# lrm2017/Fastest_Image_Pattern_Matching

Measured on AMD Instinct MI355X. Metric: template matches/sec + ms/search, 4024×3036 src ±180°; HBM GB/s vs roofline, higher is better.
Workload: dtype u8

## Files before the change

fastest_image_pattern_matching_amd/csrc/fpm_kernels.hip:

```cpp
#include <float.h>
#include <stdio.h>
#include <stdlib.h>
#include <limits.h>

#include <map>
#include <mutex>
#include <type_traits>
#include <utility>

#include "../../include/fpm.h"
#include "fpm_kernels.h"
#include "fpm_model.h"
#include "fpm_rrect.h"

static void ensure_lds_attr(const void* fn, size_t bytes) {
    if (bytes <= 65536) return;
    int dev = 0;
    (void)hipGetDevice(&dev);
    static std::mutex mu;
    static std::map<std::pair<int, const void*>, size_t> done;
    std::lock_guard<std::mutex> lock(mu);
    size_t& cur = done[std::make_pair(dev, fn)];
    if (bytes <= cur) return;
    (void)hipFuncSetAttribute(fn, hipFuncAttributeMaxDynamicSharedMemorySize, (int)bytes);
// ... 3549 lines not shown
        else { slot = item / nband; band = item - slot * nband; }
        const int T0 = band * kBandRows, rb = min(kBandRows, th - T0), nsrc = rb + 6;
        __syncthreads();
        if (NK > 0) {
            const bool in_roi = lane < 2 * txn;
            if (DMA) {
                dma_rows(item, SB);
                flush();
                asm volatile("s_waitcnt vmcnt(0)" ::: "memory");
            } else {
            if (!PFR) load_rows(item);
            flush();
#pragma unroll
            for (int i = 0; i < kStageRows; ++i) {
                const int r = wv + 4 * i;
                if (r < nsrc && lane < q4)
                    *(uint4*)(SB + (size_t)r * SBp + 16 * lane) = in_roi ? pv[i] : make_uint4(kRoiFlip, kRoiFlip, kRoiFlip, kRoiFlip);
            }
            }
            if (band != a_band) {
                a_band = band;
                if (tid < kBandRows) lts[tid] = tid < rb ? (uint32_t)a.tsum[T0 + tid] : 0u;
                if (kMmaRows * mt < rb) {
                    const int8_t* ap = a.tmpl8 + (size_t)(T0 + kMmaRows * mt + n) * a.tp8 + 16 * g;
#pragma unroll
                    for (int k = 0; k < NA; ++k)
                        if (k < a.nk) Areg[k] = *(const fpm_v4i*)(ap + 64 * k);
                }
            }
            if (PFR && item + 1 < it_hi) load_rows(item + 1);
        } else if (MODE != 3) {
            if (tid < kBandRows) lts[tid] = tid < rb ? (uint32_t)a.tsum[T0 + tid] : 0u;
            const uint8_t* rsrc = a.roi + (size_t)slot * a.roi_stride;
            for (int c0 = 0; c0 < q4; c0 += 64) {
                const int c = c0 + lane;
                for (int i0 = 0; i0 < kStageRows; i0 += kStageBatch) {
                    uint4 v[kStageBatch];
#pragma unroll
                    for (int i = 0; i < kStageBatch; ++i) {
                        const int r = wv + 4 * (i0 + i);
                        const int R = T0 + r;
                        v[i] = (r < nsrc && c < 2 * txn)
                                   ? *(const uint4*)(rsrc + ((size_t)((R >> 5) * txn + (c >> 1)) << 10) + (R & 31) * ROI_T + 16 * (c & 1))
                                   : make_uint4(kRoiFlip, kRoiFlip, kRoiFlip, kRoiFlip);
                    }
#pragma unroll
                    for (int i = 0; i < kStageBatch; ++i) {
                        const int r = wv + 4 * (i0 + i);
                        if (r < nsrc && c < q4) *(uint4*)(SB + (size_t)r * SBp + 16 * c) = v[i];
                    }
                }
            }
        }
        __syncthreads();
        if (RS >= 3 && MODE != 7 && wv != 2 && kMmaRows * nt < nsrc) {
            int ln = lane;
            asm volatile("" : "+v"(ln));
            const int g3 = ln >> 4, n3 = ln & 15, row = kMmaRows * nt + n3;
            const int sr = row < nsrc ? row : 0;
            uint32_t* rw = (uint32_t*)(SB + (size_t)sr * SBp);
            if (npad > 0) {
                if (g3 < npad) rw[nwr + g3] = kRoiFlip;
                if (g3 + 4 < npad) rw[nwr + g3 + 4] = kRoiFlip;
            }
            const int wr = tw >> 2;
            const uint32_t l0 = rw[0], l1 = rw[1], x0 = rw[wr], x1 = rw[wr + 1], x2 = rw[wr + 2];
            uint32_t s1, s2;
            tile_row_sums<RS == 4>((const uint8_t*)rw + 16 * g3, a.nk, n3, s1, s2);
            s2 = (uint32_t)__shfl((int)s2, n3 + 16 * (n3 >> 2), 64);
            const uint32_t e0 = __builtin_amdgcn_alignbyte(x1, x0, (uint32_t)tw) ^ 0x80808080u;
            const uint32_t e1 = __builtin_amdgcn_alignbyte(x2, x1, (uint32_t)tw) ^ 0x80808080u;
            const uint64_t lo = (uint64_t)(l0 ^ 0x80808080u) | ((uint64_t)(l1 ^ 0x80808080u) << 32);
            const uint64_t hi = (uint64_t)e0 | ((uint64_t)e1 << 32);
            const int nf = min(6, 64 * a.nk - tw);
#pragma unroll
            for (int h = 0; h < 2; ++h) {
                const int dx = g3 + 4 * h;
                if (dx < 7 && row < nsrc) {
                    uint32_t q1, q2;
                    window_edges(lo, hi, dx, nf, q1, q2);
                    wi[row * 7 + dx] = s1 - q1;
                    wq[row * 7 + dx] = s2 - q2;
                }
            }
        }
        if (RS == 1 && MODE != 7 && tid < 4 * nsrc) {
            const int r = tid >> 2, qq = tid & 3;
            const int per = (nwr + 3) >> 2, k0 = qq * per, k1 = min(nwr, k0 + per);
            const uint32_t* row = (const uint32_t*)(SB + (size_t)r * SBp);
            uint32_t s1 = 0, s2 = 0;
            int k = k0;
            for (; k + 8 <= k1; k += 8) {
                uint32_t x[8];
#pragma unroll
                for (int u = 0; u < 8; ++u) x[u] = row[k + u] ^ 0x80808080u;
#pragma unroll
                for (int u = 0; u < 8; ++u) {
                    s1 = __builtin_amdgcn_udot4(x[u], 0x01010101u, s1, false);
                    s2 = __builtin_amdgcn_udot4(x[u], x[u], s2, false);
                }
            }
            for (; k < k1; ++k) {
                const uint32_t x = row[k] ^ 0x80808080u;
                s1 = __builtin_amdgcn_udot4(x, 0x01010101u, s1, false);
                s2 = __builtin_amdgcn_udot4(x, x, s2, false);
            }
            const uint32_t l0 = row[0] ^ 0x80808080u, l1 = row[1] ^ 0x80808080u;
            const int wr = tw >> 2;
            const uint32_t x0 = row[wr], x1 = row[wr + 1], x2 = row[wr + 2];
            const uint32_t e0 = __builtin_amdgcn_alignbyte(x1, x0, (uint32_t)tw) ^ 0x80808080u;
            const uint32_t e1 = __builtin_amdgcn_alignbyte(x2, x1, (uint32_t)tw) ^ 0x80808080u;
            s1 += (uint32_t)__builtin_amdgcn_mov_dpp((int)s1, 0xB1, 0xF, 0xF, false);
            s2 += (uint32_t)__builtin_amdgcn_mov_dpp((int)s2, 0xB1, 0xF, 0xF, false);
            s1 += (uint32_t)__builtin_amdgcn_mov_dpp((int)s1, 0x4E, 0xF, 0xF, false);
            s2 += (uint32_t)__builtin_amdgcn_mov_dpp((int)s2, 0x4E, 0xF, 0xF, false);
#pragma unroll
            for (int h = 0; h < 2; ++h) {
                const int dx = qq + 4 * h;
                if (dx < 7) {
                    const uint32_t ml0 = dx >= 4 ? 0xffffffffu : (1u << (8 * dx)) - 1u;
                    const uint32_t ml1 = dx <= 4 ? 0u : (1u << (8 * (dx - 4))) - 1u;
                    const uint32_t mr0 = dx >= 4 ? 0u : ~((1u << (8 * dx)) - 1u);
                    const uint32_t mr1 = dx <= 4 ? 0xffffu : dx == 5 ? 0xff00u : 0u;
                    const uint32_t a0 = l0 & ml0, a1 = l1 & ml1, b0 = e0 & mr0, b1 = e1 & mr1;
                    uint32_t q1 = __builtin_amdgcn_udot4(a0, 0x01010101u, 0u, false);
                    q1 = __builtin_amdgcn_udot4(a1, 0x01010101u, q1, false);
                    q1 = __builtin_amdgcn_udot4(b0, 0x01010101u, q1, false);
                    q1 = __builtin_amdgcn_udot4(b1, 0x01010101u, q1, false);
                    uint32_t q2 = __builtin_amdgcn_udot4(a0, a0, 0u, false);
                    q2 = __builtin_amdgcn_udot4(a1, a1, q2, false);
                    q2 = __builtin_amdgcn_udot4(b0, b0, q2, false);
                    q2 = __builtin_amdgcn_udot4(b1, b1, q2, false);
                    wi[r * 7 + dx] = s1 - q1;
                    wq[r * 7 + dx] = s2 - q2;
                }
            }
        }
        __syncthreads();
        auto partials = [&]() {
            if (MODE == 6 || tid >= 4 * 49) return;
            const int pr = tid >> 1, half = tid & 1;
            const int h = pr / 49, k = pr - h * 49;
            const int chunk = (T0 >> 4) + h;
            const int tlo = kMmaRows * h, thi = min(tlo + kMmaRows, rb);
            const bool ok = chunk < a.nchunk && tlo < thi;
            const int pdy = k / 7, ddx = k - pdy * 7;
            const int t0 = tlo + 8 * half, n8 = ok ? min(8, thi - t0) : 0;
            uint32_t s1 = 0, x[8], y[8];
#pragma unroll
            for (int u = 0; u < 8; ++u) {
                const int i = (t0 + u + pdy) * 7 + ddx;
                x[u] = u < n8 ? wi[i] : 0u;
                y[u] = u < n8 ? wq[i] : 0u;
            }
            uint64_t s2 = 0;
#pragma unroll
            for (int u = 0; u < 8; ++u) { s1 += x[u]; s2 += y[u]; }
            s1 += (uint32_t)__builtin_amdgcn_mov_dpp((int)s1, 0xB1, 0xF, 0xF, false);
            const uint32_t lo = (uint32_t)s2, hi = (uint32_t)(s2 >> 32);
            s2 += (uint64_t)(uint32_t)__builtin_amdgcn_mov_dpp((int)lo, 0xB1, 0xF, 0xF, false) |
                  ((uint64_t)(uint32_t)__builtin_amdgcn_mov_dpp((int)hi, 0xB1, 0xF, 0xF, false) << 32);
            if (ok && half == 0) {
                uint32_t kk = (uint32_t)k;
                asm volatile("" : "+v"(kk));
                const uint32_t wo = ((uint32_t)slot * (uint32_t)a.nchunk + (uint32_t)chunk) * 49u + kk;
                a.wsum[wo] = s1;
                a.wsq[wo] = s2;
            }
        };
        const bool active = kMmaRows * mt < rb && kMmaRows * nt < nsrc;
        if (FPM_CORR_PRIO == 1) __builtin_amdgcn_s_setprio(1);
        if (MODE != 2 && active) {
            int sr = kMmaRows * nt + n;
            if (sr >= nsrc) sr = 0;
            const uint8_t* bp = SB + (size_t)sr * SBp + 16 * g;
            fpm_v4i acc[7];
            if (FPM_CORR_PRIO == 2) __builtin_amdgcn_s_setprio(1);
            if (NK > 0)
                band_mfma_regs<NA>(Areg, bp, a.nk, acc);
            else
                band_mfma_ga(a.tmpl8 + (size_t)(T0 + kMmaRows * mt + n) * a.tp8 + 16 * g, bp, a.nk, acc);
            if (FPM_CORR_PRIO == 2) __builtin_amdgcn_s_setprio(0);
            uint32_t* rs_out = a.rowsum + (((size_t)th * 49 + 3) & ~(size_t)3) * slot + (size_t)T0 * 49;
            const uint32_t kFix = 16384u * (uint32_t)tw;
            int t0 = kMmaRows * mt + 4 * g;
            asm volatile("" : "+v"(t0));
            const int s_ = kMmaRows * nt + n;
            const uint4 ts4 = *(const uint4*)(lts + t0);
#pragma unroll
            for (int r = 0; r < 4; ++r) {
                const int t = t0 + r, dy = s_ - t;
                if (t < rb && s_ < nsrc && dy >= 0 && dy < 7) {
                    const uint32_t ts = r == 0 ? ts4.x : r == 1 ? ts4.y : r == 2 ? ts4.z : ts4.w;
                    if (MODE == 5) {
                        uint32_t x = ts;
#pragma unroll
                        for (int d = 0; d < 7; ++d) x += (uint32_t)acc[d][r];
                        if (x == 0x9e3779b9u && a.W < 0) rs_out[t] = x;
                        continue;
                    }
                    const uint32_t o = (uint32_t)(t * 49 + dy * 7);
                    if (SE) {
#pragma unroll
                        for (int d = 0; d < 7; ++d) rsb[o + d] = (uint32_t)acc[d][r] + 128u * (wi[s_ * 7 + d] + ts) - kFix;
                        continue;
                    }
#pragma unroll
                    for (int d = 0; d < 7; ++d) rs_out[o + d] = (uint32_t)acc[d][r] + 128u * (wi[s_ * 7 + d] + ts) - kFix;
                }
            }
        }
        if (FPM_CORR_PRIO == 1) __builtin_amdgcn_s_setprio(0);
        partials();
        if (SE) { pv_slot = slot; pv_T0 = T0; pv_rb = rb; }
    }
    if (SE && pv_slot >= 0) {
        __syncthreads();
        flush();
    }
}

__device__ __forceinline__ CandState cand_step_state(CandState s, int n3, const AngleNode* nodes, double thr, int W,
                                                     int H, int mark_reached0, const float* score, const int* mx,
                                                     const int* my, const AngleNode* next_nodes = nullptr,
                                                     int jj = 0, AngleNode* next_nd = nullptr, int nnext = 1) {
    int imax = 0;
    double big = -1;
    for (int k = 0; k < n3; ++k)
        if ((double)score[k] > big) { imax = k; big = score[k]; }
    if ((double)score[imax] < thr) {
        s.alive = 0;
        return s;
    }
    const int child = s.node * n3 + imax;
    const AngleNode nd = nodes[child];
    if (next_nodes)
        for (int k = 0; k < nnext; ++k) next_nd[k] = next_nodes[child * n3 + jj + k];
    const F2 sc = f2((W - 1) / 2.0f, (H - 1) / 2.0f);
    const F2 r0 = rotate_pt(f2(s.lt.x * 2, s.lt.y * 2), sc, nd.c, nd.s);
    const F2 pad = f2(r0.x - 3, r0.y - 3);
    F2 p = f2((float)((double)mx[imax] + pad.x), (float)((double)my[imax] + pad.y));
    p = rotate_pt(p, sc, nd.cn, nd.sn);
    s.lt = p;
    s.node = child;
    s.reached0 = mark_reached0;
    return s;
}

struct SmallLayout {
    int sbp, tbp, rh, u, tab, sum, rs, sc, ts, total;
};
__host__ __device__ inline int isqrt_ceil(int n) {
    int d = 0;
    while ((d + 1) * (d + 1) <= n) ++d;
    return d * d == n ? d : d + 1;
}
__host__ __device__ inline int small_footprint_bound(int rw, int rh) {
    const int d = isqrt_ceil((rw - 1) * (rw - 1) + (rh - 1) * (rh - 1)) + 2;
    return ((d + 16) * (d + 6) + 15) & ~15;
}
__host__ __device__ inline SmallLayout small_layout(int tw, int th, int nw = 4) {
    SmallLayout L;
    L.sbp = roi_pitch_calc(tw);
    L.tbp = tmpl_lds_pitch(64 * ((tw + 63) / 64));
    L.rh = th + 6;
    const int th16 = (th + kMmaRows - 1) / kMmaRows * kMmaRows;
    L.u = ((L.rh + 16) * L.sbp + 15) & ~15;
    const int fb = small_footprint_bound(tw + 6, th + 6);
    const int fp = fb < nw * ROI_FT ? fb : nw * ROI_FT;
    const int ub = th16 * L.tbp > fp ? th16 * L.tbp : fp;
    L.tab = L.u + ub;
    L.sum = L.tab + 4 * (2 * L.sbp + 2 * ((L.rh + 3) & ~3));
    const int rs_size = 4 * kBandRows * 49;
    const int after_sums = L.sum + 4 * (2 * L.rh + 2 * 7 * L.rh) + 8 * 49 * 2;
    if (th16 * L.tbp + rs_size <= L.sum - L.u) {
        L.rs = L.u + th16 * L.tbp;
        L.sc = after_sums;
    } else {
        L.rs = after_sums;
        L.sc = L.rs + rs_size;
    }
    L.ts = L.sc + 4 * 64;
    L.total = L.ts + 4 * th16;
    return L;
}
constexpr int kSmallLdsMax = 72 * 1024;
bool roi_small_fits(int tw, int th) { return th <= 256 && small_layout(tw, th).total <= kSmallLdsMax; }
size_t roi_small_lds(int tw, int th) { return (size_t)small_layout(tw, th).total; }

template <int MODE, int WPE = 3, bool PROL = false, int NT = 256>
__global__ __launch_bounds__(NT) __attribute__((amdgpu_waves_per_eu(WPE))) void k_roi_small(RoiArgs a) {
    constexpr int NW = NT / 64;
    extern __shared__ __attribute__((aligned(16))) uint8_t smem[];
    const int tw = a.tw, th = a.th, RW = tw + 6, RH = th + 6, W = a.W, H = a.H;
    const SmallLayout LY = small_layout(tw, th, NW);
    const int SBp = LY.sbp, TBp = LY.tbp;
    uint8_t* SB = smem;
    uint8_t* TB = smem + LY.u;
    uint8_t* FTall = smem + LY.u;
    int32_t* lad = (int32_t*)(smem + LY.tab);
    int32_t* lbd = lad + SBp;
    int32_t* lx0 = lbd + SBp;
    int32_t* ly0 = lx0 + ((RH + 3) & ~3);
    uint32_t* rall = (uint32_t*)(smem + LY.sum);
    uint32_t* rallq = rall + RH;
    uint32_t* wi = rallq + RH;
    uint32_t* wq = wi + RH * 7;
    uint64_t* tot = (uint64_t*)(((uintptr_t)(wq + RH * 7) + 7) & ~(uintptr_t)7);
    uint32_t* rs = (uint32_t*)(smem + LY.rs);
    float* sc = (float*)(smem + LY.sc);
    uint32_t* lts = (uint32_t*)(smem + LY.ts);
    const int tid = threadIdx.x, lane = tid & 63, wv = tid >> 6;
    const int rois = roi_count(a);
    const int q4 = SBp >> 4, nwr = (RW + 3) >> 2;
    const int txn = (RW + ROI_T - 1) / ROI_T, tyn = (RH + ROI_T - 1) / ROI_T;
    const int g = lane >> 4, n = lane & 15;
    const int lr = lane >> 3, lg = lane & 7;
    auto STAMP = [&](int k) {
        if (MODE == 9 && tid == 0 && blockIdx.x < 64) a.stamps[blockIdx.x * 16 + k] = __builtin_readcyclecounter();
    };
    for (int slot = blockIdx.x; slot < rois; slot += gridDim.x) {
        STAMP(0);
        int id, jj;
        roi_slot(a, slot, id, jj);
        const uint8_t* lvl = a.level + (size_t)(id / a.per_source) * a.level_stride;
        CandState st = a.state[id];
        AngleNode nd;
        if (PROL) {
            if (st.alive) {
                const RoiRecord* r = a.prev_rec + (size_t)id * a.n3;
                float score[3];
                int mx[3], my[3];
                for (int k = 0; k < a.n3; ++k) { score[k] = r[k].score; mx[k] = r[k].mx; my[k] = r[k].my; }
                st = cand_step_state(st, a.n3, a.prev_nodes, a.prev_thr, a.prev_W, a.prev_H, 0, score, mx, my, a.nodes,
                                     jj, &nd);
                if (jj == 0 && tid == 0 && st.alive) atomicAdd(a.live_out_count, 1);
            }
            if (jj == 0 && tid == 0) a.state_out[id] = st;
            if (!st.alive) continue;
        } else {
            nd = a.nodes[st.node * a.n3 + jj];
        }
        __syncthreads();
        {
            double M[6];
            roi_matrix(W, H, f2(st.lt.x * 2, st.lt.y * 2), nd.c, nd.s, M);
            for (int x = tid; x < RW; x += NT) {
                lad[x] = rint_i(M[0] * x * kAbScale);
                lbd[x] = rint_i(M[3] * x * kAbScale);
            }
            for (int y = tid; y < RH; y += NT) {
                lx0[y] = rint_i((M[1] * y + M[2]) * kAbScale) + kRoundDelta;
                ly0[y] = rint_i((M[4] * y + M[5]) * kAbScale) + kRoundDelta;
            }
        }
        __syncthreads();
        STAMP(1);
        int gbx0 = INT_MAX, gbx1 = INT_MIN, gby0 = INT_MAX, gby1 = INT_MIN;
#pragma unroll
        for (int k = 0; k < 4; ++k) {
            const int c = (k & 1) ? RW - 1 : 0, r = (k & 2) ? RH - 1 : 0;
            const int X = (lx0[r] + lad[c]) >> (kAbBits - kInterBits);
            const int Y = (ly0[r] + lbd[c]) >> (kAbBits - kInterBits);
            gbx0 = min(gbx0, X >> kInterBits); gbx1 = max(gbx1, X >> kInterBits);
            gby0 = min(gby0, Y >> kInterBits); gby1 = max(gby1, Y >> kInterBits);
        }
        const bool g_interior = gbx0 - 1 >= 0 && gbx1 + 1 <= W - 2 && gby0 - 1 >= 0 && gby1 + 1 <= H - 2;
        gbx0 = max(gbx0 - 1, 0); gby0 = max(gby0 - 1, 0);
        gbx1 = min(gbx1 + 2, W - 1); gby1 = min(gby1 + 2, H - 1);
        const bool g_any = gbx0 <= gbx1 && gby0 <= gby1;
        const int gbxa = gbx0 & ~3;
        const int gftw = g_any ? ((gbx1 - gbxa + 4) & ~3) + 4 : 4;
        const int gfth = g_any ? gby1 - gby0 + 1 : 0;
        const int gobase = gby0 * gftw + gbxa;
        if (g_any && gftw * gfth <= LY.tab - LY.u) {
            uint8_t* FT = FTall;
            const int wpr = gftw >> 2;
            stage_block4(FT, gftw, lvl + (size_t)gby0 * a.P + gbxa, a.P, gfth, wpr, gbxa, a.P, tid, NT);
            __syncthreads();
            STAMP(8);
            const int ngrp = (RW + 3) >> 2;
            const int nrl = NT / ngrp;
            const int rl = tid / ngrp, c0 = 4 * (tid - rl * ngrp);
            int ad4[4], bd4[4];
#pragma unroll
            for (int u = 0; u < 4; ++u) { ad4[u] = lad[c0 + u]; bd4[u] = lbd[c0 + u]; }
            if (g_interior && MODE != 5) {
                const int xo = ((int)lds_offset_of(FT) - gbxa) << kAbBits, yo = -(gby0 << kAbBits);
                const int nvalid = RW - c0;
                const uint32_t colmask = nvalid >= 4 ? 0xffffffffu : (nvalid <= 0 ? 0u : (1u << (8 * nvalid)) - 1u);
                for (int r = rl < nrl ? rl : RH; r < RH; r += nrl) {
                    const int x0r = lx0[r] + xo, y0r = ly0[r] + yo;
                    uint32_t off[4];
                    int fxv[4], fyv[4], v[4][4];
#pragma unroll
                    for (int u = 0; u < 4; ++u) {
                        const int sxv = x0r + ad4[u], syv = y0r + bd4[u];
                        fxv[u] = __builtin_amdgcn_ubfe(sxv, kAbBits - kInterBits, kInterBits);
                        fyv[u] = __builtin_amdgcn_ubfe(syv, kAbBits - kInterBits, kInterBits);
                        off[u] = (uint32_t)mad24(syv >> kAbBits, gftw, sxv >> kAbBits);
                    }
#pragma unroll
                    for (int u = 0; u < 4; ++u) lds_taps(off[u], gftw, v[u]);
                    uint32_t pk = 0;
#pragma unroll
                    for (int u = 0; u < 4; ++u) pk |= (uint32_t)bilerp24(v[u], fxv[u], fyv[u]) << (8 * u);
                    *(uint32_t*)(SB + r * SBp + c0) = pk & colmask;
                }
            } else {
                for (int r = rl < nrl ? rl : RH; r < RH; r += nrl) {
                    const int X0 = lx0[r], Y0 = ly0[r];
                    uint32_t pk = 0;
#pragma unroll
                    for (int u = 0; u < 4; ++u) {
                        const int X = (X0 + ad4[u]) >> (kAbBits - kInterBits);
                        const int Y = (Y0 + bd4[u]) >> (kAbBits - kInterBits);
                        int v;
                        if (g_interior) {
                            const int off = mad24(Y >> kInterBits, gftw, (X >> kInterBits) - gobase);
                            v = ft_tap_bytes(FT, off, gftw, X, Y);
                        } else {
                            v = ft_tap_general(FT, gftw, gbxa, gby0, W, H, X, Y);
                        }
                        if (c0 + u >= RW) v = 0;
                        pk |= (uint32_t)v << (8 * u);
                    }
                    *(uint32_t*)(SB + r * SBp + c0) = pk;
                }
            }
            STAMP(9);
        } else if (!g_any) {
            for (int i = tid; i < RH * (SBp >> 2); i += NT) ((uint32_t*)SB)[i] = 0u;
        } else {
            const bool tile_bufs = NW * ROI_FT <= LY.tab - LY.u;
            uint8_t* FT = FTall + wv * ROI_FT;
            for (int task = wv; task < txn * tyn; task += NW) {
                const int ty = task / txn, tx = task - ty * txn;
                const int cx0 = tx * ROI_T, cx1 = min(cx0 + ROI_T, RW) - 1;
                const int ry0 = ty * ROI_T, ry1 = min(ry0 + ROI_T, RH) - 1;
                int bx0 = INT_MAX, bx1 = INT_MIN, by0 = INT_MAX, by1 = INT_MIN;
#pragma unroll
                for (int k = 0; k < 4; ++k) {
                    const int c = (k & 1) ? cx1 : cx0, r = (k & 2) ? ry1 : ry0;
                    const int X = (lx0[r] + lad[c]) >> (kAbBits - kInterBits);
                    const int Y = (ly0[r] + lbd[c]) >> (kAbBits - kInterBits);
                    bx0 = min(bx0, X >> kInterBits); bx1 = max(bx1, X >> kInterBits);
                    by0 = min(by0, Y >> kInterBits); by1 = max(by1, Y >> kInterBits);
                }
                const bool interior = bx0 - 1 >= 0 && bx1 + 1 <= W - 2 && by0 - 1 >= 0 && by1 + 1 <= H - 2;
                bx0 = max(bx0 - 1, 0); by0 = max(by0 - 1, 0);
                bx1 = min(bx1 + 2, W - 1); by1 = min(by1 + 2, H - 1);
                const bool any = bx0 <= bx1 && by0 <= by1;
                const int bxa = bx0 & ~3;
                int ftw = any ? ((bx1 - bxa + 4) & ~3) : 0;
                if (((ftw >> 2) & 1) == 0) ftw += 4;
                const int fth = any ? by1 - by0 + 1 : 0;
                const int wpr = ftw >> 2;
                const bool in_lds = tile_bufs && wpr <= 16 && ftw * fth <= ROI_FT;
                wave_sync();
                if (any && in_lds) stage_footprint<4>(FT, ftw, wpr, fth, lvl + (size_t)by0 * a.P + bxa, a.P, bxa, a.P, lane);
                wave_sync();
                const int c0 = cx0 + 4 * lg;
                if (c0 > cx1) continue;
                for (int i = 0; i < 4; ++i) {
                    const int r = ry0 + lr + 8 * i;
                    if (r > ry1) break;
                    const int X0 = lx0[r], Y0 = ly0[r];
                    uint32_t pk = 0;
#pragma unroll
                    for (int u = 0; u < 4; ++u) {
                        const int X = (X0 + lad[c0 + u]) >> (kAbBits - kInterBits);
                        const int Y = (Y0 + lbd[c0 + u]) >> (kAbBits - kInterBits);
                        int v;
                        if (interior && in_lds) {
                            const int off = mad24(Y >> kInterBits, ftw, (X >> kInterBits) - (by0 * ftw + bxa));
                            v = MODE == 5 ? ft_tap_bytes(FT, off, ftw, X, Y) : ft_tap_interior(FT, off, ftw, X, Y);
                        } else {
                            v = in_lds ? ft_tap_general(FT, ftw, bxa, by0, W, H, X, Y) : roi_tap(lvl, W, H, a.P, X, Y);
                        }
                        if (c0 + u >= RW) v = 0;
                        pk |= (uint32_t)v << (8 * u);
                    }
                    *(uint32_t*)(SB + r * SBp + c0) = pk;
                }
            }
        }
        __syncthreads();
        if (MODE == 1) continue;
        STAMP(2);
        for (int r = tid; r < RH; r += NT) {
            const uint32_t* row = (const uint32_t*)(SB + (size_t)r * SBp);
            uint32_t s1 = 0, s2 = 0;
            int k = 0;
            for (; k + 8 <= nwr; k += 8) {
                uint32_t x[8];
#pragma unroll
                for (int u = 0; u < 8; ++u) x[u] = row[k + u];
#pragma unroll
                for (int u = 0; u < 8; ++u) {
                    s1 = __builtin_amdgcn_udot4(x[u], 0x01010101u, s1, false);
                    s2 = __builtin_amdgcn_udot4(x[u], x[u], s2, false);
                }
            }
            for (; k < nwr; ++k) {
                const uint32_t x = row[k];
                s1 = __builtin_amdgcn_udot4(x, 0x01010101u, s1, false);
                s2 = __builtin_amdgcn_udot4(x, x, s2, false);
            }
            rall[r] = s1;
            rallq[r] = s2;
        }
        __syncthreads();
        for (int i = tid; i < RH * q4; i += NT) {
            uint4* v = (uint4*)SB + i;
            uint4 x = *v;
            x.x ^= 0x80808080u; x.y ^= 0x80808080u; x.z ^= 0x80808080u; x.w ^= 0x80808080u;
            *v = x;
        }
        {
            const int trows = (th + kMmaRows - 1) / kMmaRows * kMmaRows;
            stage_block16(TB, TBp, (const uint8_t*)a.tmpl8, a.tp8, trows, a.tp8 >> 4, tid, NT);
            if (WPE < 4)
                for (int i = tid; i < (NT >= 256 ? min(trows, NT) : trows); i += NT) lts[i] = (uint32_t)a.tsum[i];
        }
        __syncthreads();
        STAMP(3);
        for (int r = tid; r < RH; r += NT) {
            const uint8_t* sbr = SB + (size_t)r * SBp;
            uint32_t lv[6], rv[6];
#pragma unroll
            for (int c = 0; c < 6; ++c) { lv[c] = sbr[c] ^ 0x80u; rv[c] = sbr[tw + c] ^ 0x80u; }
            uint32_t q1 = rall[r], q2 = rallq[r];
#pragma unroll
            for (int c = 0; c < 6; ++c) { q1 -= rv[c]; q2 -= rv[c] * rv[c]; }
#pragma unroll
            for (int dx = 0; dx < 7; ++dx) {
                if (dx > 0) {
                    q1 += rv[dx - 1] - lv[dx - 1];
                    q2 += rv[dx - 1] * rv[dx - 1] - lv[dx - 1] * lv[dx - 1];
                }
                wi[r * 7 + dx] = q1;
                wq[r * 7 + dx] = q2;
            }
        }
        if (tid < 98) tot[tid] = 0;
        __syncthreads();
        STAMP(4);
#pragma unroll 1
        for (int q = tid; q < (NT >= 4 * 49 ? (tid < 4 * 49 ? tid + 1 : 0) : 4 * 49); q += NT) {
            const int part = q / 49, k = q - part * 49, pdy = k / 7, ddx = k - pdy * 7;
            const int t0 = part * th / 4, t1 = (part + 1) * th / 4;
            uint64_t s1 = 0, s2 = 0;
            int t = t0;
            for (; t + 8 <= t1; t += 8) {
                uint32_t x[8], y[8];
#pragma unroll
                for (int u = 0; u < 8; ++u) { x[u] = wi[(t + u + pdy) * 7 + ddx]; y[u] = wq[(t + u + pdy) * 7 + ddx]; }
#pragma unroll
                for (int u = 0; u < 8; ++u) { s1 += x[u]; s2 += y[u]; }
            }
            for (; t < t1; ++t) { s1 += wi[(t + pdy) * 7 + ddx]; s2 += wq[(t + pdy) * 7 + ddx]; }
            atomicAdd((unsigned long long*)&tot[k], (unsigned long long)s1);
            atomicAdd((unsigned long long*)&tot[49 + k], (unsigned long long)s2);
        }
        if (MODE == 2) continue;
        STAMP(5);
        float accF = 0.f;
        uint64_t accI = 0;
        const uint32_t kFix = 16384u * (uint32_t)tw;
        for (int T0 = 0; T0 < th; T0 += kBandRows) {
            const int rb = min(kBandRows, th - T0), nsrc = rb + 6;
#pragma unroll
            for (int pass = 0; pass < (4 + NW - 1) / NW; ++pass) {
            const int p = wv + pass * NW, mt = p & 1, nt = mt + (p >> 1);
            if (p < 4 && kMmaRows * mt < rb && kMmaRows * nt < nsrc) {
                const uint8_t* ap = TB + (size_t)(T0 + kMmaRows * mt + n) * TBp + 16 * g;
                const uint8_t* bp = SB + (size_t)(T0 + kMmaRows * nt + n) * SBp + 16 * g;
                fpm_v4i acc[7];
                band_mfma(ap, bp, a.nk, acc);
                const int s_ = kMmaRows * nt + n;
#pragma unroll
                for (int r = 0; r < 4; ++r) {
                    const int t = kMmaRows * mt + 4 * g + r, dy = s_ - t;
                    if (t < rb && s_ < nsrc && dy >= 0 && dy < 7) {
                        const uint32_t ts = WPE < 4 ? lts[T0 + t] : (uint32_t)a.tsum[T0 + t];
#pragma unroll
                        for (int d = 0; d < 7; ++d)
                            rs[t * 49 + dy * 7 + d] = (uint32_t)acc[d][r] + 128u * (wi[(T0 + s_) * 7 + d] + ts) - kFix;
                    }
                }
            }
            }
            __syncthreads();
            if (MODE != 3 && tid < 49) {
                if (a.fold) {
                    int t = 0;
                    for (; t + 8 <= rb; t += 8) {
                        uint32_t x[8];
#pragma unroll
                        for (int u = 0; u < 8; ++u) x[u] = rs[(t + u) * 49 + tid];
#pragma unroll
                        for (int u = 0; u < 8; ++u) accF = accF + (float)(int)x[u];
                    }
                    for (; t < rb; ++t) accF = accF + (float)(int)rs[t * 49 + tid];
                } else {
                    for (int t = 0; t < rb; ++t) accI += rs[t * 49 + tid];
                }
            }
            __syncthreads();
        }
        if (tid < 49) {
            const double num = a.fold ? (double)accF : (double)(float)(double)accI;
            sc[tid] = ccoeff(num, (double)tot[tid], (double)tot[49 + tid], a.mean, a.norm, a.inv_area);
        }
        __syncthreads();
        STAMP(6);
        if (wv == 0) {
            float v = lane < 49 ? sc[lane] : -INFINITY;
            int bi = lane < 49 ? lane : 64;
            if (v != v) { v = -INFINITY; bi = 64 + lane; }
            wave_better_reduce(v, bi);
            const float s0 = sc[0];
            if (s0 != s0 || bi >= 64) bi = 0;
            const float best = sc[bi];
            const int mx = bi % 7, my = bi / 7;
            RoiRecord r;
            r.score = best;
            r.mx = (int16_t)mx;
            r.my = (int16_t)my;
            const int border = (mx == 0 || my == 0 || mx == 6 || my == 6) ? 1 : 0;
            r.on_border = border;
            for (int x = -1; x <= 1; ++x)
                for (int y = -1; y <= 1; ++y) r.vec[(x + 1) * 3 + (y + 1)] = border ? 0.f : sc[(my + y) * 7 + (mx + x)];
            if (lane == 0) a.rec[(size_t)id * a.n3 + jj] = r;
        }
        STAMP(7);
    }
}

__device__ int cand_step_one(const RoiArgs& a, int id, const float* score, const int* mx, const int* my,
                             CandState* so = nullptr, AngleNode* nn = nullptr) {
    CandState* out = a.state_out ? a.state_out : a.state;
    CandState s = a.state[id];
    if (!s.alive) {
        out[id] = s;
        return -1;
    }
    s = cand_step_state(s, a.n3, a.nodes, a.thr, a.W, a.H, a.mark_reached0, score, mx, my, nn ? a.nt_nodes : nullptr,
                        0, nn, a.n3);
    out[id] = s;
    if (so) *so = s;
    if (!s.alive) return -1;
    const int p = atomicAdd(a.live_out_count, 1);
    a.live_out[p] = id;
    return p;
}

__device__ __forceinline__ void cand_next_tables(const RoiArgs& a, int id, int p, const CandState& s,
                                                 const AngleNode& nd, int j, int lane) {
    roi_tables_fill(a.nt_tab, a.tdesc, a.tdesc_stride, a.nt_tabw, a.nt_tabh, a.nt_tw, a.nt_th, a.nt_W, a.nt_H,
                    p * a.n3 + j, s.lt, nd, (id / a.per_source) << kTileSrcShift, lane, 64);
}

__global__ __launch_bounds__(256) void k_cand_step(RoiArgs a) {
    const int n = *a.live_count;
    for (int li = blockIdx.x * 256 + threadIdx.x; li < n; li += gridDim.x * 256) {
        const int id = a.live[li];
        const RoiRecord* r = a.rec + (size_t)id * a.n3;
        float score[3];
        int mx[3], my[3];
        for (int k = 0; k < a.n3; ++k) { score[k] = r[k].score; mx[k] = r[k].mx; my[k] = r[k].my; }
        cand_step_one(a, id, score, mx, my);
    }
}

__global__ __launch_bounds__(192) void k_cand_step_tab(RoiArgs a) {
    __shared__ int pos;
    __shared__ CandState ns;
    __shared__ AngleNode nn[3];
    const int n = *a.live_count;
    const int lane = threadIdx.x & 63, j = threadIdx.x >> 6;
    for (int li = blockIdx.x; li < n; li += gridDim.x) {
        const int id = a.live[li];
        __syncthreads();
        if (threadIdx.x == 0) {
            const RoiRecord* r = a.rec + (size_t)id * a.n3;
            float score[3];
            int mx[3], my[3];
            for (int k = 0; k < a.n3; ++k) { score[k] = r[k].score; mx[k] = r[k].mx; my[k] = r[k].my; }
            CandState s;
            pos = cand_step_one(a, id, score, mx, my, &s, a.nt_tab ? nn : nullptr);
            ns = s;
        }
        __syncthreads();
        if (pos >= 0 && j < a.n3) cand_next_tables(a, id, pos, ns, nn[j], j, lane);
    }
}

template <int ROWS>
struct EvalBlk {
    static_assert(ROWS * 49 % 4 == 0, "a block is whole uint4 of the [th][49] series");
    static constexpr int dma = (ROWS * 49 / 4 + 63) / 64;
    static constexpr int buf = dma * 1024;
};

template <int ROWS>
__device__ void eval_roi(const RoiArgs& a, int slot, int lane, uint8_t* blk, float* sc, RoiRecord* out,
                         RoiRecord* keep) {
    constexpr int kEvalRows = ROWS, kEvalDma = EvalBlk<ROWS>::dma, kEvalBuf = EvalBlk<ROWS>::buf;
    const int th = a.th;
    if (a.equal1) {
        if (lane == 0) {
            RoiRecord r;
            r.score = 1.f; r.mx = 0; r.my = 0; r.on_border = 1;
            for (int k = 0; k < 9; ++k) r.vec[k] = 0.f;
            *out = r;
            *keep = r;
        }
        return;
    }
    const size_t total4 = ((size_t)th * 49 + 3) >> 2;
    const uint4* rs = (const uint4*)(a.rowsum + (size_t)slot * total4 * 4);
    uint64_t s1 = 0, s2 = 0;
    if (lane < 49) {
        const uint32_t* ws = a.wsum + (size_t)slot * a.nchunk * 49 + lane;
        const uint64_t* wq = a.wsq + (size_t)slot * a.nchunk * 49 + lane;
        int c = 0;
        for (; c + 8 <= a.nchunk; c += 8) {
            uint32_t x[8];
            uint64_t y[8];
#pragma unroll
            for (int u = 0; u < 8; ++u) { x[u] = ws[(size_t)(c + u) * 49]; y[u] = wq[(size_t)(c + u) * 49]; }
#pragma unroll
            for (int u = 0; u < 8; ++u) { s1 += x[u]; s2 += y[u]; }
        }
        for (; c < a.nchunk; ++c) { s1 += ws[(size_t)c * 49]; s2 += wq[(size_t)c * 49]; }
    }
    constexpr int BQ = kEvalRows * 49 / 4;
    const int nblk = (th + kEvalRows - 1) / kEvalRows;
    auto issue_block = [&](int b, uint8_t* buf) {
#pragma unroll
        for (int i = 0; i < kEvalDma; ++i) {
            size_t q = (size_t)b * BQ + 64 * i + lane;
            if (64 * i + lane >= BQ || q >= total4) q = 0;
            uint32_t keep;
            const uint32_t ldsa = (uint32_t)(uintptr_t)(fpm_lds_vp)(buf + 1024 * i);
            asm volatile("s_mov_b32 %0, m0\n\ts_mov_b32 m0, %2\n\ts_nop 0\n\tglobal_load_lds_dwordx4 %1, off\n\ts_mov_b32 m0, %0"
                         : "=&s"(keep) : "v"(rs + q), "s"(__builtin_amdgcn_readfirstlane(ldsa)) : "memory");
        }
    };
    float accF = 0.f;
    uint64_t accI = 0;
    issue_block(0, blk);
    for (int b = 0; b < nblk; ++b) {
        const uint32_t* cb = (const uint32_t*)(blk + (b & 1) * kEvalBuf);
        if (b + 1 < nblk) {
            issue_block(b + 1, blk + ((b + 1) & 1) * kEvalBuf);
            asm volatile("s_waitcnt vmcnt(%0)" :: "i"(kEvalDma) : "memory");
        } else {
            asm volatile("s_waitcnt vmcnt(0)" ::: "memory");
        }
        wave_sync();
        const int rows = min(kEvalRows, th - b * kEvalRows);
        if (lane < 49) {
            if (a.fold) {
                int t = 0;
                for (; t + 8 <= rows; t += 8) {
                    uint32_t x[8];
#pragma unroll
                    for (int u = 0; u < 8; ++u) x[u] = cb[(t + u) * 49 + lane];
#pragma unroll
                    for (int u = 0; u < 8; ++u) accF = accF + (float)(int)x[u];
                }
                for (; t < rows; ++t) accF = accF + (float)(int)cb[t * 49 + lane];
            } else {
                for (int t = 0; t < rows; ++t) accI += cb[t * 49 + lane];
            }
        }
        wave_sync();
    }
    if (lane < 49) {
        const double num = a.fold ? (double)accF : (double)(float)(double)accI;
        sc[lane] = ccoeff(num, (double)s1, (double)s2, a.mean, a.norm, a.inv_area);
    }
    wave_sync();
    if (lane == 0) {
        float best = sc[0];
        int bi = 0;
        for (int k = 1; k < 49; ++k)
            if (sc[k] > best) { best = sc[k]; bi = k; }
        const int mx = bi % 7, my = bi / 7;
        RoiRecord r;
        r.score = best;
        r.mx = (int16_t)mx;
        r.my = (int16_t)my;
        const int border = (mx == 0 || my == 0 || mx == 6 || my == 6) ? 1 : 0;
        r.on_border = border;
        for (int x = -1; x <= 1; ++x)
            for (int y = -1; y <= 1; ++y) r.vec[(x + 1) * 3 + (y + 1)] = border ? 0.f : sc[(my + y) * 7 + (mx + x)];
        *out = r;
        *keep = r;
    }
}

template <int ROWS>
__global__ __launch_bounds__(192) void k_roi_eval(RoiArgs a) {
    __shared__ __attribute__((aligned(16))) uint8_t blk_all[3][2 * EvalBlk<ROWS>::buf];
    __shared__ float sc_all[3][64];
    __shared__ RoiRecord recs[3];
    __shared__ int pos;
    __shared__ CandState ns;
    __shared__ AngleNode nn[3];
    const int lane = threadIdx.x & 63, j = threadIdx.x >> 6;
    const int rois = roi_count(a);
    const int base = roi_base(a);
    const int c_lo = base / a.n3, c_hi = (base + rois) / a.n3;
    for (int li = c_lo + blockIdx.x; li < c_hi; li += gridDim.x) {
        const int id = a.live[li];
        const int slot = li * a.n3 + j - base;
        __syncthreads();
        eval_roi<ROWS>(a, slot, lane, blk_all[j], sc_all[j], a.rec + (size_t)id * a.n3 + j, &recs[j]);
        if (!a.step) continue;
        __syncthreads();
        if (threadIdx.x == 0) {
            float score[3];
            int mx[3], my[3];
            for (int k = 0; k < a.n3; ++k) { score[k] = recs[k].score; mx[k] = recs[k].mx; my[k] = recs[k].my; }
            CandState s;
            pos = cand_step_one(a, id, score, mx, my, &s, a.nt_tab ? nn : nullptr);
            ns = s;
        }
        if (!a.nt_tab) continue;
        __syncthreads();
        if (pos >= 0) cand_next_tables(a, id, pos, ns, nn[j], j, lane);
    }
}

void launch_roi_tables(const RoiArgs& a, hipStream_t st) {
    if (a.slot_cap <= 0 || a.equal1) return;
    const int grid = a.slot_cap < 4096 ? a.slot_cap : 4096;
    hipLaunchKernelGGL(k_roi_tables, dim3(grid), dim3(256), 0, st, a);
}

constexpr int kWarpFootBatch = 12, kWarpWaves = 8;
static int grid_cap_env(const char* v, int dflt) { return v ? (atoi(v) > 0 ? atoi(v) : 0) : dflt; }
static int capped(int grid, int cap) { return cap > 0 && grid > cap ? cap : grid; }
// ... 652 lines not shown
```

Measured before the change: 36320.

## Fuse ROI row sums with window sums and write pre-flipped bytes

The ROI sampling stage now writes bytes already XORed with the sign-flip constant, which removes the separate pass that flipped the whole ROI buffer in LDS. The per-row sum and sum-of-squares pass is merged with the 7-wide window-sum pass. It also splits each row across 2 or 4 lanes and combines the partial sums with DPP swizzles, which drops the rall/rallq scratch arrays and two barriers. The cost is an extra XOR on every load in the row-sum loop and more complex lane indexing. The code relies on kRoiFlip being defined elsewhere and equal to 0x80808080.

```diff
diff --git a/fastest_image_pattern_matching_amd/csrc/fpm_kernels.hip b/fastest_image_pattern_matching_amd/csrc/fpm_kernels.hip
--- a/fastest_image_pattern_matching_amd/csrc/fpm_kernels.hip
+++ b/fastest_image_pattern_matching_amd/csrc/fpm_kernels.hip
@@ -3875,9 +3875,7 @@
     int32_t* lbd = lad + SBp;
     int32_t* lx0 = lbd + SBp;
     int32_t* ly0 = lx0 + ((RH + 3) & ~3);
-    uint32_t* rall = (uint32_t*)(smem + LY.sum);
-    uint32_t* rallq = rall + RH;
-    uint32_t* wi = rallq + RH;
+    uint32_t* wi = (uint32_t*)(smem + LY.sum) + 2 * RH;
     uint32_t* wq = wi + RH * 7;
     uint64_t* tot = (uint64_t*)(((uintptr_t)(wq + RH * 7) + 7) & ~(uintptr_t)7);
     uint32_t* rs = (uint32_t*)(smem + LY.rs);
@@ -3885,7 +3883,7 @@
     uint32_t* lts = (uint32_t*)(smem + LY.ts);
     const int tid = threadIdx.x, lane = tid & 63, wv = tid >> 6;
     const int rois = roi_count(a);
-    const int q4 = SBp >> 4, nwr = (RW + 3) >> 2;
+    const int nwr = (RW + 3) >> 2;
     const int txn = (RW + ROI_T - 1) / ROI_T, tyn = (RH + ROI_T - 1) / ROI_T;
     const int g = lane >> 4, n = lane & 15;
     const int lr = lane >> 3, lg = lane & 7;
@@ -3978,7 +3976,7 @@
                     uint32_t pk = 0;
 #pragma unroll
                     for (int u = 0; u < 4; ++u) pk |= (uint32_t)bilerp24(v[u], fxv[u], fyv[u]) << (8 * u);
-                    *(uint32_t*)(SB + r * SBp + c0) = pk & colmask;
+                    *(uint32_t*)(SB + r * SBp + c0) = (pk & colmask) ^ kRoiFlip;
                 }
             } else {
                 for (int r = rl < nrl ? rl : RH; r < RH; r += nrl) {
@@ -3998,12 +3996,12 @@
                         if (c0 + u >= RW) v = 0;
                         pk |= (uint32_t)v << (8 * u);
                     }
-                    *(uint32_t*)(SB + r * SBp + c0) = pk;
+                    *(uint32_t*)(SB + r * SBp + c0) = pk ^ kRoiFlip;
                 }
             }
             STAMP(9);
         } else if (!g_any) {
-            for (int i = tid; i < RH * (SBp >> 2); i += NT) ((uint32_t*)SB)[i] = 0u;
+            for (int i = tid; i < RH * (SBp >> 2); i += NT) ((uint32_t*)SB)[i] = kRoiFlip;
         } else {
             const bool tile_bufs = NW * ROI_FT <= LY.tab - LY.u;
             uint8_t* FT = FTall + wv * ROI_FT;
@@ -4054,67 +4052,67 @@
                         if (c0 + u >= RW) v = 0;
                         pk |= (uint32_t)v << (8 * u);
                     }
-                    *(uint32_t*)(SB + r * SBp + c0) = pk;
+                    *(uint32_t*)(SB + r * SBp + c0) = pk ^ kRoiFlip;
                 }
             }
         }
         __syncthreads();
         if (MODE == 1) continue;
         STAMP(2);
-        for (int r = tid; r < RH; r += NT) {
-            const uint32_t* row = (const uint32_t*)(SB + (size_t)r * SBp);
-            uint32_t s1 = 0, s2 = 0;
-            int k = 0;
-            for (; k + 8 <= nwr; k += 8) {
-                uint32_t x[8];
-#pragma unroll
-                for (int u = 0; u < 8; ++u) x[u] = row[k + u];
-#pragma unroll
-                for (int u = 0; u < 8; ++u) {
-                    s1 = __builtin_amdgcn_udot4(x[u], 0x01010101u, s1, false);
-                    s2 = __builtin_amdgcn_udot4(x[u], x[u], s2, false);
-                }
-            }
-            for (; k < nwr; ++k) {
-                const uint32_t x = row[k];
-                s1 = __builtin_amdgcn_udot4(x, 0x01010101u, s1, false);
-                s2 = __builtin_amdgcn_udot4(x, x, s2, false);
-            }
-            rall[r] = s1;
-            rallq[r] = s2;
-        }
-        __syncthreads();
-        for (int i = tid; i < RH * q4; i += NT) {
-            uint4* v = (uint4*)SB + i;
-            uint4 x = *v;
-            x.x ^= 0x80808080u; x.y ^= 0x80808080u; x.z ^= 0x80808080u; x.w ^= 0x80808080u;
-            *v = x;
-        }
+        {
+            const int lsh = 4 * RH <= NT ? 2 : 1, nl = 1 << lsh, ql = tid & (nl - 1);
+            for (int r0 = 0; r0 < RH; r0 += NT >> lsh) {
+                const int r = r0 + (tid >> lsh);
+                const uint8_t* sbr = SB + (size_t)min(r, RH - 1) * SBp;
+                const uint32_t* row = (const uint32_t*)sbr;
+                uint32_t s1 = 0, s2 = 0;
+                int k = ql;
+                for (; k + 3 * nl < nwr; k += 4 * nl) {
+                    uint32_t x[4];
+#pragma unroll
+                    for (int u = 0; u < 4; ++u) x[u] = row[k + u * nl] ^ kRoiFlip;
+#pragma unroll
+                    for (int u = 0; u < 4; ++u) {
+                        s1 = __builtin_amdgcn_udot4(x[u], 0x01010101u, s1, false);
+                        s2 = __builtin_amdgcn_udot4(x[u], x[u], s2, false);
+                    }
+                }
+                for (; k < nwr; k += nl) {
+                    const uint32_t x = row[k] ^ kRoiFlip;
+                    s1 = __builtin_amdgcn_udot4(x, 0x01010101u, s1, false);
+                    s2 = __builtin_amdgcn_udot4(x, x, s2, false);
+                }
+                s1 += (uint32_t)__builtin_amdgcn_mov_dpp((int)s1, 0xB1, 0xF, 0xF, false);
+                s2 += (uint32_t)__builtin_amdgcn_mov_dpp((int)s2, 0xB1, 0xF, 0xF, false);
+                if (lsh == 2) {
+                    s1 += (uint32_t)__builtin_amdgcn_mov_dpp((int)s1, 0x4E, 0xF, 0xF, false);
+                    s2 += (uint32_t)__builtin_amdgcn_mov_dpp((int)s2, 0x4E, 0xF, 0xF, false);
+                }
+                if (ql == 0 && r < RH) {
+                    uint32_t lv[6], rv[6];
+#pragma unroll
+                    for (int c = 0; c < 6; ++c) { lv[c] = sbr[c] ^ 0x80u; rv[c] = sbr[tw + c] ^ 0x80u; }
+                    uint32_t q1 = s1, q2 = s2;
+#pragma unroll
+                    for (int c = 0; c < 6; ++c) { q1 -= rv[c]; q2 -= rv[c] * rv[c]; }
+#pragma unroll
+                    for (int dx = 0; dx < 7; ++dx) {
+                        if (dx > 0) {
+                            q1 += rv[dx - 1] - lv[dx - 1];
+                            q2 += rv[dx - 1] * rv[dx - 1] - lv[dx - 1] * lv[dx - 1];
+                        }
+                        wi[r * 7 + dx] = q1;
+                        wq[r * 7 + dx] = q2;
+                    }
+                }
+            }
+        }
+        STAMP(3);
         {
             const int trows = (th + kMmaRows - 1) / kMmaRows * kMmaRows;
             stage_block16(TB, TBp, (const uint8_t*)a.tmpl8, a.tp8, trows, a.tp8 >> 4, tid, NT);
             if (WPE < 4)
                 for (int i = tid; i < (NT >= 256 ? min(trows, NT) : trows); i += NT) lts[i] = (uint32_t)a.tsum[i];
-        }
-        __syncthreads();
-        STAMP(3);
-        for (int r = tid; r < RH; r += NT) {
-            const uint8_t* sbr = SB + (size_t)r * SBp;
-            uint32_t lv[6], rv[6];
-#pragma unroll
-            for (int c = 0; c < 6; ++c) { lv[c] = sbr[c] ^ 0x80u; rv[c] = sbr[tw + c] ^ 0x80u; }
-            uint32_t q1 = rall[r], q2 = rallq[r];
-#pragma unroll
-            for (int c = 0; c < 6; ++c) { q1 -= rv[c]; q2 -= rv[c] * rv[c]; }
-#pragma unroll
-            for (int dx = 0; dx < 7; ++dx) {
-                if (dx > 0) {
-                    q1 += rv[dx - 1] - lv[dx - 1];
-                    q2 += rv[dx - 1] * rv[dx - 1] - lv[dx - 1] * lv[dx - 1];
-                }
-                wi[r * 7 + dx] = q1;
-                wq[r * 7 + dx] = q2;
-            }
         }
         if (tid < 98) tot[tid] = 0;
         __syncthreads();
```

New measurement: 36580 (median of 6 runs). No clear change (+0.7%).
